# stecrotti/MPSKit.jl

Hardware: AMD Instinct MI355X
Metric: DMRG sweeps/sec + ddAC matvec achieved-TFLOP/s, Heisenberg L=100 D=1024 fp64 (higher is better)
Workload: dtype f64; 1 GPU; Heisenberg S=1/2 FiniteMPS L=100 D=1024 d=2 W=5 fp64, 1-site DMRG sweep (2L-2 site updates), fixed Krylov budget 8 matvecs/site; parallelism=single GPU

## Files before the change

mpskit.jl_amd/csrc/mpsk_api.hip:

```cpp
#include <hip/hip_runtime.h>
#include <cstdio>
#include <cstdlib>
#include <cstring>
#include <cmath>
#include <algorithm>
#include <map>
#include <string>
#include <vector>
#include "mpsk.h"
#include "mpsk_internal.h"

using namespace mpsk;

static thread_local std::string g_err;
static int fail(int code, const std::string& msg) { g_err = msg; return code; }
#define HIPCHK(expr)                                                                        \
  do {                                                                                      \
    hipError_t e_ = (expr);                                                                 \
    if (e_ != hipSuccess)                                                                   \
      return fail(MPSK_ERR_HIP, std::string(#expr) + ": " + hipGetErrorString(e_));         \
  } while (0)
#define REQUIRE(cond, msg)                                                  \
  do {                                                                      \
    if (!(cond)) return fail(MPSK_ERR_INVALID, std::string(__func__) + ": " + (msg)); \
// ... 12 lines not shown
  MixPlan rgt;
  double Oi(int w, int t, int s, int v) const {
    return Ofull_im.empty() ? 0.0 : Ofull_im[w + (size_t)Wl * (t + d * (s + (size_t)d * v))];
  }
  std::vector<char> row_used, col_used;
  MixPlan rc;
  std::vector<int> rc_w, rc_s, rc_t;
  int rc_nseg = 0;
  bool jordan = false;
  MixPlan jr, jl;
  std::vector<int> jr_p, jl_p;
  int jr_nseg = 0, jl_nseg = 0;
  MixPlan tl, tr;
  bool tl_dblock = false;
  mutable std::map<int64_t, int64_t*> jtabL;
  mutable std::map<std::pair<int64_t, int64_t>, int64_t*> jtabR;
  double O(int w, int t, int s, int v) const { return Ofull[w + (size_t)Wl * (t + d * (s + (size_t)d * v))]; }
  bool dense = false;
  double* d_Od = nullptr;
  mutable std::map<std::pair<int64_t, int64_t>, int64_t*> dtab;
  double* d_OdR = nullptr;
  mutable std::map<std::pair<int64_t, int64_t>, int64_t*> dtabR;
};

struct PoolBuf { void* p; size_t bytes; bool used; hipStream_t last = nullptr; hipEvent_t ev = nullptr; bool ev_set = false; };

struct mpsk_ctx {
  int device = 0;
  hipStream_t stream = nullptr;
  void* ws = nullptr;
  size_t ws_bytes = 0;
  double* d_scal = nullptr;
  double* d_partial = nullptr;
  double* h_scal = nullptr;
  double* d_coef = nullptr;
  double* h_coef = nullptr;
  hipEvent_t ev_coef = nullptr;
  bool coef_pending = false;
  int dtype = MPSK_F64;
  int last_svd_sweeps = 0;
  int split_skip = 0, split_backoff = 0;
  std::map<std::pair<int, int>, int> split_q_hint;
  int last_split_iters = 0, last_split_path = 0;
  double last_split_resid = 0.0;
  int svd_precondition = 3;
  int qr_mode = 0;
  int* d_flag = nullptr;
  long n_qr_chol = 0, n_qr_house = 0, n_qr_fallback = 0, n_qr_robust = 0, n_qr_retry = 0;
  double qr_shift_fast = getenv("MPSK_CQ_SHIFT_SCALE") ? atof(getenv("MPSK_CQ_SHIFT_SCALE")) : 1.0e-8;
  hipStream_t stream2 = nullptr;
  hipStream_t xstreams[3] = {nullptr, nullptr, nullptr};
  hipEvent_t ev_fork = nullptr, ev_join = nullptr;
  void* ws2 = nullptr;
  size_t ws2_bytes = 0;
  void* ws3 = nullptr;
  size_t ws3_bytes = 0;
  void* cxws[4] = {nullptr, nullptr, nullptr, nullptr};
  size_t cxws_bytes[4] = {0, 0, 0, 0};
  int* h_flags = nullptr;
  struct PendingQR {
    int active = 0;
    int m = 0, n = 0;
    const void *A1 = nullptr, *A2 = nullptr; void *Q1 = nullptr, *R1 = nullptr, *Q2 = nullptr, *R2 = nullptr;
    int lda1 = 0, ldq1 = 0, ldr1 = 0, lda2 = 0, ldq2 = 0, ldr2 = 0;
    double *At = nullptr, *Qt = nullptr, *Rt = nullptr, *ws = nullptr;
    void *L = nullptr, *Qo = nullptr; int ldl = 0, ldqo = 0;
// ... 15 lines not shown
  const double* GL;
  const double* GR;
  int mode;
  double* GRc = nullptr;
  double* GLc = nullptr;
  int launches = 1;
  int64_t* zseg = nullptr;
  std::vector<int64_t> zseg_host;
  hipEvent_t ev_up = nullptr;
  int pool_idx = -1;
};
constexpr int MAXK = 256;
constexpr int MAXCOEF = 1024;

extern "C" {

int mpsk_version(void) { return 100; }
const char* mpsk_last_error(void) { return g_err.c_str(); }

int mpsk_ctx_create(int device, mpsk_ctx** out) {
  REQUIRE(out != nullptr, "out is NULL");
  int ndev = 0;
  HIPCHK(hipGetDeviceCount(&ndev));
  REQUIRE(device >= 0 && device < ndev, "no such HIP device (is a GPU visible?)");
  HIPCHK(hipSetDevice(device));
  hipDeviceProp_t prop;
  HIPCHK(hipGetDeviceProperties(&prop, device));
  if (std::strncmp(prop.gcnArchName, "gfx950", 6) != 0)
    return fail(MPSK_ERR_UNSUPPORTED, std::string("libmpsk is built for gfx950 only, device is ") + prop.gcnArchName);
  mpsk_ctx* c = new mpsk_ctx();
  c->device = device;
  HIPCHK(hipMalloc(&c->d_scal, sizeof(double) * MAXK));
  HIPCHK(hipMalloc(&c->d_partial, sizeof(double) * MPSK_DOT_SCRATCH));
  HIPCHK(hipHostMalloc(&c->h_scal, sizeof(double) * MAXK, hipHostMallocDefault));
  HIPCHK(hipMalloc(&c->d_coef, sizeof(double) * MAXCOEF));
  HIPCHK(hipHostMalloc(&c->h_coef, sizeof(double) * MAXCOEF, hipHostMallocDefault));
  HIPCHK(hipEventCreateWithFlags(&c->ev_coef, hipEventDisableTiming | hipEventDisableSystemFence));
  HIPCHK(hipMalloc(&c->d_flag, 64));
  HIPCHK(hipHostMalloc(&c->h_flags, 64, hipHostMallocDefault));
  HIPCHK(hipStreamCreateWithFlags(&c->stream2, hipStreamNonBlocking));
  c->xstreams[0] = c->stream2;
  HIPCHK(hipStreamCreateWithFlags(&c->xstreams[1], hipStreamNonBlocking));
  HIPCHK(hipStreamCreateWithFlags(&c->xstreams[2], hipStreamNonBlocking));
  HIPCHK(hipEventCreateWithFlags(&c->ev_fork, hipEventDisableTiming | hipEventDisableSystemFence));
  HIPCHK(hipEventCreateWithFlags(&c->ev_join, hipEventDisableTiming | hipEventDisableSystemFence));
  gemm_retain_stream(c->stream);
  gemm_retain_stream(c->stream2);
  gemm_retain_stream(c->xstreams[1]);
  gemm_retain_stream(c->xstreams[2]);
  *out = c;
  return MPSK_OK;
}

int mpsk_ctx_destroy(mpsk_ctx* c) {
  if (!c) return MPSK_OK;
  (void)hipSetDevice(c->device);
  if (c->on_side) (void)mpsk_ctx_side_end(c);
  if (c->pend.active) (void)mpsk_qr_commit(c, nullptr);
  (void)hipStreamSynchronize(c->stream);
  if (c->stream2) (void)hipStreamSynchronize(c->stream2);
  gemm_release_stream(c->stream);
  gemm_release_stream(c->stream2);
  for (auto& kv : c->pair_plans) mix_plan_destroy(&kv.second);
  for (auto& b : c->pool) { if (b.p) (void)hipFree(b.p); if (b.ev) (void)hipEventDestroy(b.ev); }
  if (c->ws) (void)hipFree(c->ws);
  if (c->d_scal) (void)hipFree(c->d_scal);
  if (c->d_partial) (void)hipFree(c->d_partial);
  if (c->h_scal) (void)hipHostFree(c->h_scal);
  if (c->d_coef) (void)hipFree(c->d_coef);
  if (c->h_coef) (void)hipHostFree(c->h_coef);
  if (c->ev_coef) (void)hipEventDestroy(c->ev_coef);
  if (c->d_flag) (void)hipFree(c->d_flag);
  if (c->h_flags) (void)hipHostFree(c->h_flags);
  if (c->ws2) (void)hipFree(c->ws2);
  if (c->ws3) (void)hipFree(c->ws3);
  if (c->exws) (void)hipFree(c->exws);
  for (auto& kv : c->prod_tabs) (void)hipFree(kv.second);
  for (int i = 0; i < 4; ++i) if (c->cxws[i]) (void)hipFree(c->cxws[i]);
  for (int i = 1; i < 3; ++i)
    if (c->xstreams[i]) { (void)hipStreamSynchronize(c->xstreams[i]); gemm_release_stream(c->xstreams[i]); (void)hipStreamDestroy(c->xstreams[i]); }
  if (c->stream2) { (void)hipStreamSynchronize(c->stream2); (void)hipStreamDestroy(c->stream2); }
  if (c->ev_fork) (void)hipEventDestroy(c->ev_fork);
  if (c->ev_join) (void)hipEventDestroy(c->ev_join);
  delete c;
  return MPSK_OK;
}

int mpsk_ctx_set_stream(mpsk_ctx* c, void* s) {
  REQUIRE(c, "ctx is NULL");
  REQUIRE(!c->on_side, "not inside a side-stream section (mpsk_ctx_side_end first)");
  REQUIRE(!c->pend.active, "a deferred factorization is pending (mpsk_qr_commit first)");
  if (c->stream != (hipStream_t)s) {
    (void)hipSetDevice(c->device);
    (void)hipStreamSynchronize(c->stream);
    gemm_release_stream(c->stream);
    gemm_retain_stream((hipStream_t)s);
  }
  c->stream = (hipStream_t)s;
  return MPSK_OK;
}
// ... 969 lines not shown
  const bool cplx = h->H->dtype == MPSK_C128;
  const bool shift = a0[0] != 0.0 || (cplx && a0[1] != 0.0);
  const bool scale = a1[0] != 1.0 || (cplx && a1[1] != 0.0);
  REQUIRE(!shift || (h->Dlo == h->Dl && nblk == 1), "a shift needs a square operator (Dlo == Dl) on the plain vector layout");
  if (int rc = mpsk_hac_apply(h, x, nblk, y)) return rc;
  if (!shift && !scale) return MPSK_OK;
  mpsk_ctx* c = h->ctx;
  const int64_t n = (int64_t)h->Dlo * h->H->d * h->Dr;
  if (cplx) {
    HIPCHK(vec_axpby_c(a0, shift ? (const double*)x : nullptr, a1, (double*)y, n, c->stream));
  } else if (shift) {
    HIPCHK(vec_axpby(a0[0], (const double*)x, a1[0], (double*)y, n, c->stream));
  } else {
    HIPCHK(vec_scal(a1[0], (double*)y, n, c->stream));
  }
  return MPSK_OK;
}

int mpsk_hac_eigsolve_fixed(mpsk_hac* h, const void* x0, int m, void* const* V, void* scal, void* y, void* first_image) {
  REQUIRE(h && x0 && V && scal && y, "NULL argument");
  REQUIRE(m >= 1 && m <= 32, "needs 1 <= m <= 32");
  REQUIRE(h->H->dtype == MPSK_F64, "mpsk_hac_eigsolve_fixed: MPSK_F64 operators only");
  mpsk_ctx* c = h->ctx;
  HIPCHK(hipSetDevice(c->device));
  const int64_t n = (int64_t)h->Dlo * h->H->d * h->Dr;
  REQUIRE(h->Dlo == h->Dl, "mpsk_hac_eigsolve_fixed: the operator must be square (unsharded)");
  double* slot = (double*)scal;
  const int stride = 2 * m + 1;
  double* rbuf = slot + (size_t)m * stride;
  if (int rc = mpsk_vnormalize_dev(c, n, x0, V[0], nullptr)) return rc;
  for (int k = 0; k < m; ++k) {
    if (int rc = mpsk_hac_apply(h, V[k], 1, V[k + 1])) return rc;
    if (k == 0 && first_image) HIPCHK(hipMemcpyAsync(first_image, V[1], sizeof(double) * n, hipMemcpyDeviceToDevice, c->stream));
    HIPCHK(vec_cgs2((const double* const*)V, k + 1, (double*)V[k + 1], n, slot + (size_t)k * stride, c->d_partial, c->stream));
    HIPCHK(vec_scal_rsqrt_dev(slot + (size_t)k * stride + 2 * (k + 1), (double*)V[k + 1], n, c->stream));
  }
  HIPCHK(vec_ritz_small(slot, m, stride, rbuf, rbuf + 32, c->stream));
  HIPCHK(hipMemsetAsync(V[m + 1], 0, sizeof(double) * n, c->stream));
  HIPCHK(vec_multiaxpy((const double* const*)V, rbuf, m, 1.0, (double*)V[m + 1], n, c->stream));
  return mpsk_vnormalize_dev(c, n, V[m + 1], y, nullptr);
}

int mpsk_dC(mpsk_ctx* c, int W, int Dlo, int Dl, int Dr, const void* GL, const void* GR, const void* cm, void* y) {
  REQUIRE(c && GL && GR && cm && y, "NULL argument");
  REQUIRE(W > 0 && Dlo > 0 && Dl > 0 && Dr > 0, "dimensions must be positive");
  if (c->dtype == MPSK_C128)
    return dC_c128(c, W, Dlo, Dl, Dr, (const double*)GL, (const double*)GR, (const double*)cm, (double*)y);
  HIPCHK(hipSetDevice(c->device));
  const size_t slab = (size_t)Dlo * Dr;
  if (int rc = ensure_ws(c, sizeof(double) * slab * W)) return rc;
  double* T1 = (double*)c->ws;
  GemmArgs g1 = mk((const double*)GL, (const double*)cm, T1, Dlo, Dr, Dl, Dlo, Dl, Dlo);
  g1.batch = W; g1.bsA = (int64_t)Dlo * Dl; g1.bsB = 0; g1.bsC = (int64_t)slab;
  g1.tag = 1;
  HIPCHK(gemm_f64(g1, c->stream));
  std::vector<int64_t> sa, sb;
  for (int w = 0; w < W; ++w) { sa.push_back((int64_t)w * slab); sb.push_back((int64_t)w * Dr * Dr); }
  GemmArgs g3 = mk(T1, (const double*)GR, (double*)y, Dlo, Dr, Dr, Dlo, Dr, Dlo);
  g3.tag = 1;
  HIPCHK(gemm_segments(g3, sa, sb, c->stream));
  return MPSK_OK;
}

static int pair_plan(mpsk_ctx* c, const mpsk_mposlice* H1, const mpsk_mposlice* H2, const MixPlan** out) {
  auto key = std::make_pair(H1, H2);
  auto it = c->pair_plans.find(key);
  if (it != c->pair_plans.end()) { *out = &it->second; return MPSK_OK; }
  const int d1 = H1->d, d2 = H2->d, Wl = H1->Wl, Wm = H1->Wr, Wr = H2->Wr;
// ... 1417 lines not shown

int mpsk_vnrm2(mpsk_ctx* c, int64_t n, const void* x, double* host_out) {
  double v = 0.0;
  if (int rc = mpsk_vdot(c, n, x, x, &v)) return rc;
  *host_out = std::sqrt(v);
  return MPSK_OK;
}

int mpsk_vdiff_nrm2(mpsk_ctx* c, int64_t n, const void* x, const void* y, double* host_out) {
  REQUIRE(c && x && y && host_out, "NULL argument");
  REQUIRE(n > 0, "bad n");
  REQUIRE(((uintptr_t)x % 16 == 0) && ((uintptr_t)y % 16 == 0), "operands must be 16-byte aligned");
  HIPCHK(hipSetDevice(c->device));
  HIPCHK(vec_diff_nrm2((const double*)x, (const double*)y, c->dtype == MPSK_C128 ? 2 * n : n, c->d_scal, c->d_partial,
                       c->stream));
  return fetch_scalars(c, 2, host_out);
}

int mpsk_vgs_step(mpsk_ctx* c, int64_t n, int k, const void* const* xs, void* y, double* host_out) {
  REQUIRE(c && xs && y && host_out, "NULL argument");
  REQUIRE(k > 0 && k <= MAXK && n > 0, "bad k or n");
  HIPCHK(hipSetDevice(c->device));
  HIPCHK(vec_multidot((const double* const*)xs, k, (const double*)y, n, c->d_scal, c->d_partial, c->stream));
  HIPCHK(vec_multiaxpy((const double* const*)xs, c->d_scal, k, -1.0, (double*)y, n, c->stream));
  return fetch_scalars(c, k, host_out);
}

int mpsk_vorth_step(mpsk_ctx* c, int64_t n, int k, const void* const* xs, void* y, double* host_h, double* host_beta) {
  REQUIRE(c && xs && y && host_h && host_beta, "NULL argument");
  REQUIRE(k > 0 && 2 * k + 1 <= MAXK && n > 0, "bad k or n");
  HIPCHK(hipSetDevice(c->device));
  const double* const* X = (const double* const*)xs;
  double* yy = (double*)y;
  HIPCHK(vec_cgs2(X, k, yy, n, c->d_scal, c->d_partial, c->stream));
  HIPCHK(vec_scal_rsqrt_dev(c->d_scal + 2 * k, yy, n, c->stream));
  double tmp[MAXK];
  if (int rc = fetch_scalars(c, 2 * k + 1, tmp)) return rc;
  for (int j = 0; j < k; ++j) host_h[j] = tmp[j] + tmp[k + j];
  *host_beta = tmp[2 * k] > 0.0 ? std::sqrt(tmp[2 * k]) : 0.0;
  return MPSK_OK;
}

int mpsk_vorth_step_dev(mpsk_ctx* c, int64_t n, int k, const void* const* xs, void* y, void* dev_out) {
  REQUIRE(c && xs && y && dev_out, "NULL argument");
  REQUIRE(k > 0 && 2 * k + 1 <= MAXK && n > 0, "bad k or n");
  HIPCHK(hipSetDevice(c->device));
  const double* const* X = (const double* const*)xs;
  double* yy = (double*)y;
  double* out = (double*)dev_out;
  HIPCHK(vec_cgs2(X, k, yy, n, out, c->d_partial, c->stream));
  HIPCHK(vec_scal_rsqrt_dev(out + 2 * k, yy, n, c->stream));
  return MPSK_OK;
}

int mpsk_vlincomb(mpsk_ctx* c, int64_t n, int k, const void* const* xs, const double* host_coefs, void* y) {
  REQUIRE(c && xs && y && host_coefs, "NULL argument");
  REQUIRE(k > 0 && k <= MAXK && n > 0, "bad k or n");
  HIPCHK(hipSetDevice(c->device));
  if (c->coef_pending) { HIPCHK(hipEventSynchronize(c->ev_coef)); c->coef_pending = false; }
  std::memcpy(c->h_coef, host_coefs, sizeof(double) * k);
  HIPCHK(hipMemcpyAsync(c->d_coef, c->h_coef, sizeof(double) * k, hipMemcpyHostToDevice, c->stream));
  HIPCHK(hipEventRecord(c->ev_coef, c->stream));
  c->coef_pending = true;
  HIPCHK(hipMemsetAsync(y, 0, sizeof(double) * n, c->stream));
  HIPCHK(vec_multiaxpy((const double* const*)xs, c->d_coef, k, 1.0, (double*)y, n, c->stream));
  return MPSK_OK;
}

int mpsk_vmultilincomb(mpsk_ctx* c, int64_t n, int k, const void* const* xs, int m, void* const* ys, const double* host_coefs) {
  REQUIRE(c && xs && ys && host_coefs, "NULL argument");
  REQUIRE(k > 0 && k <= 32 && m > 0 && m <= 32 && n > 0, "needs 0 < k, m <= 32 and n > 0");
  for (int j = 0; j < m; ++j)
    for (int i = 0; i < k; ++i) REQUIRE(ys[j] != xs[i], "outputs must not alias inputs");
  HIPCHK(hipSetDevice(c->device));
  if (c->coef_pending) { HIPCHK(hipEventSynchronize(c->ev_coef)); c->coef_pending = false; }
  std::memcpy(c->h_coef, host_coefs, sizeof(double) * (size_t)k * m);
  HIPCHK(hipMemcpyAsync(c->d_coef, c->h_coef, sizeof(double) * (size_t)k * m, hipMemcpyHostToDevice, c->stream));
  HIPCHK(hipEventRecord(c->ev_coef, c->stream));
  c->coef_pending = true;
  HIPCHK(vec_multilincomb((const double* const*)xs, k, (double* const*)ys, m, c->d_coef, n, c->stream));
  return MPSK_OK;
}

int mpsk_vritz_dev(mpsk_ctx* c, int m, int stride, const void* dev_slot, void* dev_coef, void* dev_info) {
  REQUIRE(c && dev_slot && dev_coef, "NULL argument");
  REQUIRE(m > 0 && m <= 32 && stride >= 2 * m + 1, "needs 0 < m <= 32 and stride >= 2 m + 1");
  HIPCHK(hipSetDevice(c->device));
  HIPCHK(vec_ritz_small((const double*)dev_slot, m, stride, (double*)dev_coef, (double*)dev_info, c->stream));
  return MPSK_OK;
}

int mpsk_vlincomb_dev(mpsk_ctx* c, int64_t n, int k, const void* const* xs, const void* dev_coefs, void* y) {
  REQUIRE(c && xs && y && dev_coefs, "NULL argument");
  REQUIRE(k > 0 && k <= MAXK && n > 0, "bad k or n");
  HIPCHK(hipSetDevice(c->device));
  HIPCHK(hipMemsetAsync(y, 0, sizeof(double) * n, c->stream));
  HIPCHK(vec_multiaxpy((const double* const*)xs, (const double*)dev_coefs, k, 1.0, (double*)y, n, c->stream));
  return MPSK_OK;
}

int mpsk_vnormalize_dev(mpsk_ctx* c, int64_t n, const void* x, void* y, void* dev_n2) {
  REQUIRE(c && x && y, "NULL argument");
  REQUIRE(n > 0, "bad n");
  HIPCHK(hipSetDevice(c->device));
  double* n2 = dev_n2 ? (double*)dev_n2 : c->d_scal + (MAXK - 1);
  const double* xs[1] = {(const double*)x};
  HIPCHK(vec_multidot(xs, 1, (const double*)x, n, n2, c->d_partial, c->stream));
  if (y != x) HIPCHK(vec_scal_rsqrt_dev_oop(n2, (const double*)x, (double*)y, n, c->stream));
  else HIPCHK(vec_scal_rsqrt_dev(n2, (double*)y, n, c->stream));
  return MPSK_OK;
}

int mpsk_vnrm2_dev(mpsk_ctx* c, int64_t n, const void* x, void* dev_out) {
  REQUIRE(c && x && dev_out, "NULL argument");
  REQUIRE(n > 0, "bad n");
  HIPCHK(hipSetDevice(c->device));
  const double* xs[1] = {(const double*)x};
  HIPCHK(vec_multidot(xs, 1, (const double*)x, n, (double*)dev_out, c->d_partial, c->stream));
  return MPSK_OK;
}

int mpsk_vaxpby(mpsk_ctx* c, int64_t n, double alpha, const void* x, double beta, void* y) {
  REQUIRE(c && x && y, "NULL argument");
  HIPCHK(hipSetDevice(c->device));
  HIPCHK(vec_axpby(alpha, (const double*)x, beta, (double*)y, n, c->stream));
  return MPSK_OK;
}
static bool aligned16(const void* p) { return (uintptr_t)p % 16 == 0; }

int mpsk_vdotc(mpsk_ctx* c, int64_t n, const void* x, const void* y, double* host_out) {
  REQUIRE(c && x && y && host_out, "NULL argument");
  REQUIRE(n > 0, "bad n");
  REQUIRE(aligned16(x) && aligned16(y), "operands must be 16-byte aligned");
  HIPCHK(hipSetDevice(c->device));
  const double* xs[1] = {(const double*)x};
  HIPCHK(vec_multidotc(xs, 1, (const double*)y, n, c->d_scal, c->d_partial, c->stream));
  return fetch_scalars(c, 2, host_out);
}

int mpsk_vaxpby_c(mpsk_ctx* c, int64_t n, const double* alpha, const void* x, const double* beta, void* y) {
  REQUIRE(c && x && y && alpha && beta, "NULL argument");
  REQUIRE(n > 0, "bad n");
// ... 359 lines not shown
```

mpskit.jl_amd/csrc/mpsk_internal.h:

```cpp
#pragma once
#include <hip/hip_runtime.h>
#include <stdint.h>
#include <stddef.h>
#include <atomic>
#include <vector>
#include <string>

namespace mpsk {

inline hipError_t ensure_dyn_smem(std::atomic<uint64_t>& done, const void* kernel, size_t bytes) {
  int dev = 0;
  hipError_t e = hipGetDevice(&dev);
  if (e != hipSuccess) return e;
  const uint64_t bit = 1ull << (dev & 63);
  if (done.load(std::memory_order_acquire) & bit) return hipSuccess;
  e = hipFuncSetAttribute(kernel, hipFuncAttributeMaxDynamicSharedMemorySize, (int)bytes);
  if (e != hipSuccess) return e;
  done.fetch_or(bit, std::memory_order_release);
  return hipSuccess;
}

constexpr int MAXSEG = 32;

struct GemmArgs {
// ... 59 lines not shown

struct MixTerm { int32_t out, in; double coef; double coef_im = 0.0; };

struct MixPlan {
  int n_out = 0, n_in = 0;
  int32_t* d_rowptr = nullptr;
  int32_t* d_src = nullptr;
  double* d_coef = nullptr;
  double* d_coef_im = nullptr;
  int nnz = 0;
  int max_terms = 0;
};

hipError_t mix_plan_create(const std::vector<MixTerm>& terms, int n_out, int n_in, MixPlan* plan);
void mix_plan_destroy(MixPlan* plan);

struct SlabIndex { int n0, n1; int64_t s0, s1, s2; int64_t ld; };
hipError_t mix_apply(const MixPlan& plan, const double* in, SlabIndex iin, double* out, SlabIndex iout,
                     int R, int C, hipStream_t s);
hipError_t deinterleave(const double* z, int64_t n, double* re, double* im, hipStream_t s);
hipError_t copy_strided(const double* src, int64_t srs, int64_t scs, double* dst, int64_t drs, int64_t dcs, int64_t R,
                        int64_t C, hipStream_t s);
hipError_t identity_slab(double* G, int n, hipStream_t s);

constexpr int MPSK_DOT_SCRATCH = 32 * 1024;
hipError_t vec_multidot(const double* const* xs, int k, const double* y, int64_t n, double* d_out,
                        double* d_partial, hipStream_t s);
hipError_t vec_diff_nrm2(const double* x, const double* y, int64_t n, double* d_out, double* d_partial, hipStream_t s);
hipError_t vec_axpby(double a, const double* x, double b, double* y, int64_t n, hipStream_t s);
hipError_t vec_times_i(const double* x, double* y, int64_t n, hipStream_t s);
hipError_t vec_scal(double a, double* x, int64_t n, hipStream_t s);
hipError_t vec_scal_rsqrt_dev(const double* d_n2, double* x, int64_t n, hipStream_t s);
hipError_t vec_scal_rsqrt_dev_oop(const double* d_n2, const double* x, double* y, int64_t n, hipStream_t s);
hipError_t vec_cgs2(const double* const* xs, int k, double* y, int64_t n, double* d_out, double* d_partial, hipStream_t s);
hipError_t vec_ritz_small(const double* d_slot, int m, int stride, double* d_coef, double* d_info, hipStream_t s);
hipError_t vec_multilincomb(const double* const* xs, int k, double* const* ys, int m, const double* d_coefs, int64_t n,
                            hipStream_t s);
hipError_t vec_multiaxpy(const double* const* xs, const double* d_coefs, int k, double sign, double* y,
                         int64_t n, hipStream_t s);
hipError_t vec_multidotc(const double* const* xs, int k, const double* y, int64_t n, double* d_out, double* d_partial,
                         hipStream_t s);
hipError_t vec_multiaxpy_c(const double* const* xs, const double* d_coefs, int k, double sign, double* y, int64_t n,
                           hipStream_t s);
hipError_t vec_cgs2_c(const double* const* xs, int k, double* y, int64_t n, double* d_out, double* d_partial, hipStream_t s);
hipError_t vec_axpby_c(const double a[2], const double* x, const double b[2], double* y, int64_t n, hipStream_t s);
hipError_t identity_dev_c(const double* G, int n, double* d_out, int nblocks, hipStream_t s);

size_t regularize_workspace_doubles(int W, int D1, int D2);
hipError_t regularize(int W, int D1, int D2, double* v, const double* lvec, const double* rvec, double* partial, hipStream_t s);
hipError_t transpose(const double* in, int ldi, int rows, int cols, double* out, int ldo, hipStream_t s);
size_t qrpos_workspace_doubles(int m, int n);
hipError_t qrpos(int m, int n, const double* A, int lda, double* Q, int ldq, double* R, int ldr, double* ws,
                 hipStream_t s, std::string* err);

size_t cholqr_workspace_doubles(int m, int n);
hipError_t cholqr3(int m, int n, const double* A, int lda, double* Q, int ldq, double* R, int ldr, double* ws,
                   int* d_flag, int* flag_out, hipStream_t s, double shift_scale = 1.0);
hipError_t cholqr_robust(int m, int n, const double* A, int lda, double* Q, int ldq, double* R, int ldr, double* ws,
                         int* d_flag, int* flag_out, hipStream_t s);
hipError_t cholqr1_orth(int m, int n, const double* X, int ldx, double* Q, int ldq, double* ws, int* d_flag, hipStream_t s,
                        double shift_scale);
hipError_t cholqr3_enqueue(int m, int n, const double* A, int lda, double* Q, int ldq, double* R, int ldr, double* ws,
                           int* d_flag, int* flag_out, hipStream_t s, double shift_scale = 1.0);
hipError_t cholqr3_finalize(int m, int n, double* Q, int ldq, double* R, int ldr, double* ws, int* d_flag,
                            int* flag_out, hipStream_t s);
size_t tsvd_workspace_bytes(int m, int n);
hipError_t tsvd(int m, int n, const double* theta, int ldt, double* U, int ldu, double* S, double* Vh, int ldv,
// ... 10 lines not shown
```

mpskit.jl_amd/csrc/mpsk_ops.hip:

```cpp
#include <hip/hip_runtime.h>
#include "mpsk_internal.h"

namespace mpsk {

typedef double d2 __attribute__((ext_vector_type(2)));

__device__ inline int64_t slab_off(const SlabIndex& ix, int j) {
  int j0 = j % ix.n0;
  int t = j / ix.n0;
  int j1 = t % ix.n1;
  int j2 = t / ix.n1;
  return j0 * ix.s0 + j1 * ix.s1 + j2 * ix.s2;
}

template <bool VEC2>
__global__ __launch_bounds__(256) void mix_kernel(const int32_t* __restrict__ rowptr,
                                                  const int32_t* __restrict__ src,
                                                  const double* __restrict__ coef,
                                                  const double* __restrict__ coef_im,
                                                  const double* __restrict__ in, SlabIndex iin,
                                                  double* __restrict__ out, SlabIndex iout, int R, int C) {
  const int o = blockIdx.y;
  const int t0 = rowptr[o], t1 = rowptr[o + 1];
  double* op = out + slab_off(iout, o);
  if (VEC2) {
    const int R2 = R >> 1;
    const int64_t total = (int64_t)R2 * C;
    for (int64_t e = blockIdx.x * (int64_t)blockDim.x + threadIdx.x; e < total;
         e += (int64_t)gridDim.x * blockDim.x) {
      int r = (int)(e % R2) * 2, c = (int)(e / R2);
      d2 acc = {0.0, 0.0};
      if (coef_im) {
        for (int t = t0; t < t1; ++t) {
// ... 172 lines not shown
    for (int j = 0; j < NVEC; ++j) {
      d2 xv = *reinterpret_cast<const d2*>(xs.p[j] + 2 * e);
      acc[j] += xv.x * yv.x + xv.y * yv.y;
    }
  }
  if ((n & 1) && blockIdx.x == 0 && threadIdx.x == 0) {
#pragma unroll
    for (int j = 0; j < NVEC; ++j) acc[j] += xs.p[j][n - 1] * y[n - 1];
  }
  block_sum<NVEC>(acc, sh);
  if (threadIdx.x == 0) {
#pragma unroll
    for (int j = 0; j < NVEC; ++j) partial[(int64_t)j * DOT_BLOCKS + blockIdx.x] = acc[j];
  }
}

__global__ __launch_bounds__(256) void dot_final_kernel(const double* __restrict__ partial, int nblocks,
                                                        double* __restrict__ out) {
  __shared__ double sh[4];
  double acc[1] = {0.0};
  const double* p = partial + (int64_t)blockIdx.x * DOT_BLOCKS;
  for (int i = threadIdx.x; i < nblocks; i += blockDim.x) acc[0] += p[i];
  block_sum<1>(acc, sh);
  if (threadIdx.x == 0) out[blockIdx.x] = acc[0];
}

static int dot_grid(int64_t n) {
  int64_t b = (n / 2 + 255) / 256;
  if (b < 1) b = 1;
  if (b > DOT_BLOCKS) b = DOT_BLOCKS;
  return (int)b;
}

hipError_t vec_multidot(const double* const* xs, int k, const double* y, int64_t n, double* d_out,
                        double* d_partial, hipStream_t s) {
  const int nb = dot_grid(n);
  for (int j0 = 0; j0 < k; j0 += MD) {
    int nv = k - j0 < MD ? k - j0 : MD;
    PtrPack pk;
    for (int j = 0; j < MD; ++j) pk.p[j] = xs[j0 + (j < nv ? j : 0)];
    switch (nv) {
      case 1: hipLaunchKernelGGL(multidot_kernel<1>, dim3(nb), dim3(256), 0, s, pk, y, n, d_partial); break;
      case 2: hipLaunchKernelGGL(multidot_kernel<2>, dim3(nb), dim3(256), 0, s, pk, y, n, d_partial); break;
      case 3: hipLaunchKernelGGL(multidot_kernel<3>, dim3(nb), dim3(256), 0, s, pk, y, n, d_partial); break;
      case 4: hipLaunchKernelGGL(multidot_kernel<4>, dim3(nb), dim3(256), 0, s, pk, y, n, d_partial); break;
      case 5: hipLaunchKernelGGL(multidot_kernel<5>, dim3(nb), dim3(256), 0, s, pk, y, n, d_partial); break;
      case 6: hipLaunchKernelGGL(multidot_kernel<6>, dim3(nb), dim3(256), 0, s, pk, y, n, d_partial); break;
      case 7: hipLaunchKernelGGL(multidot_kernel<7>, dim3(nb), dim3(256), 0, s, pk, y, n, d_partial); break;
      default: hipLaunchKernelGGL(multidot_kernel<8>, dim3(nb), dim3(256), 0, s, pk, y, n, d_partial); break;
    }
    hipLaunchKernelGGL(dot_final_kernel, dim3(nv), dim3(256), 0, s, d_partial, nb, d_out + j0);
  }
  return hipGetLastError();
}

__global__ __launch_bounds__(256) void diff_nrm2_kernel(const double* __restrict__ x, const double* __restrict__ y, int64_t n,
                                                        double* __restrict__ partial) {
  __shared__ double sh[4 * 2];
  double acc[2] = {0.0, 0.0};
  const int64_t n2 = n >> 1;
  for (int64_t e = blockIdx.x * (int64_t)blockDim.x + threadIdx.x; e < n2; e += (int64_t)gridDim.x * blockDim.x) {
    const d2 xv = *reinterpret_cast<const d2*>(x + 2 * e);
    const d2 yv = *reinterpret_cast<const d2*>(y + 2 * e);
    const double d0 = xv.x - yv.x, d1 = xv.y - yv.y;
    acc[0] += d0 * d0 + d1 * d1;
    acc[1] += xv.x * xv.x + xv.y * xv.y;
// ... 47 lines not shown
  if ((n & 1) && blockIdx.x == 0 && threadIdx.x == 0) {
    double v = y[n - 1];
#pragma unroll
    for (int j = 0; j < NVEC; ++j) v += c[j] * xs.p[j][n - 1];
    y[n - 1] = v;
    if (NORM) acc[0] += v * v;
    else {
#pragma unroll
      for (int j = 0; j < NVEC; ++j) acc[NORM ? 0 : j] += xs.p[j][n - 1] * v;
    }
  }
  block_sum<NA>(acc, sh);
  if (threadIdx.x == 0) {
#pragma unroll
    for (int j = 0; j < NA; ++j) partial[(int64_t)j * DOT_BLOCKS + blockIdx.x] = acc[j];
  }
}

template <bool NORM>
static void launch_axpy_dot(int nv, int nb, const PtrPack& pk, const double* cf, double sign, double* y, int64_t n,
                            double* d_partial, hipStream_t s) {
  switch (nv) {
    case 1: hipLaunchKernelGGL((multiaxpy_dot_kernel<1, NORM>), dim3(nb), dim3(256), 0, s, pk, cf, sign, y, n, d_partial); break;
    case 2: hipLaunchKernelGGL((multiaxpy_dot_kernel<2, NORM>), dim3(nb), dim3(256), 0, s, pk, cf, sign, y, n, d_partial); break;
    case 3: hipLaunchKernelGGL((multiaxpy_dot_kernel<3, NORM>), dim3(nb), dim3(256), 0, s, pk, cf, sign, y, n, d_partial); break;
    case 4: hipLaunchKernelGGL((multiaxpy_dot_kernel<4, NORM>), dim3(nb), dim3(256), 0, s, pk, cf, sign, y, n, d_partial); break;
    case 5: hipLaunchKernelGGL((multiaxpy_dot_kernel<5, NORM>), dim3(nb), dim3(256), 0, s, pk, cf, sign, y, n, d_partial); break;
    case 6: hipLaunchKernelGGL((multiaxpy_dot_kernel<6, NORM>), dim3(nb), dim3(256), 0, s, pk, cf, sign, y, n, d_partial); break;
    case 7: hipLaunchKernelGGL((multiaxpy_dot_kernel<7, NORM>), dim3(nb), dim3(256), 0, s, pk, cf, sign, y, n, d_partial); break;
    default: hipLaunchKernelGGL((multiaxpy_dot_kernel<8, NORM>), dim3(nb), dim3(256), 0, s, pk, cf, sign, y, n, d_partial); break;
  }
}

constexpr int ML = 32;
struct PtrPackL { const double* p[ML]; };

template <int NVEC>
__global__ __launch_bounds__(256) void multiaxpy_dot_long_kernel(PtrPackL xs, const double* __restrict__ coefs, double sign,
                                                                 double* __restrict__ y, int64_t n, int k,
                                                                 double* __restrict__ partial) {
  __shared__ double sh[4 * NVEC];
  double c[NVEC], acc[NVEC];
#pragma unroll
  for (int j = 0; j < NVEC; ++j) { c[j] = j < k ? sign * coefs[j] : 0.0; acc[j] = 0.0; }
  for (int64_t e = blockIdx.x * (int64_t)blockDim.x + threadIdx.x; e < n; e += (int64_t)gridDim.x * blockDim.x) {
    double yv = y[e];
    double xv[NVEC];
#pragma unroll
    for (int j = 0; j < NVEC; ++j) {
      xv[j] = xs.p[j][e];
      yv += c[j] * xv[j];
    }
    y[e] = yv;
#pragma unroll
    for (int j = 0; j < NVEC; ++j) acc[j] += xv[j] * yv;
  }
  block_sum<NVEC>(acc, sh);
  if (threadIdx.x == 0) {
#pragma unroll
    for (int j = 0; j < NVEC; ++j)
      if (j < k) partial[(int64_t)j * DOT_BLOCKS + blockIdx.x] = acc[j];
  }
}

__global__ __launch_bounds__(256) void multiaxpy_norm_long_kernel(PtrPackL xs, const double* __restrict__ coefs, double sign,
                                                                  double* __restrict__ y, int64_t n, int k,
                                                                  double* __restrict__ partial) {
  __shared__ double sh[4];
  __shared__ double cs[ML];
  if (threadIdx.x < ML) cs[threadIdx.x] = threadIdx.x < k ? sign * coefs[threadIdx.x] : 0.0;
  __syncthreads();
  double acc[1] = {0.0};
  for (int64_t e = blockIdx.x * (int64_t)blockDim.x + threadIdx.x; e < n; e += (int64_t)gridDim.x * blockDim.x) {
    double yv = y[e];
    for (int j = 0; j < k; ++j) yv += cs[j] * xs.p[j][e];
    y[e] = yv;
    acc[0] += yv * yv;
  }
  block_sum<1>(acc, sh);
  if (threadIdx.x == 0) partial[blockIdx.x] = acc[0];
}

static int dot_grid_long(int64_t n) {
  int64_t b = (n + 255) / 256;
  if (b < 1) b = 1;
  if (b > DOT_BLOCKS) b = DOT_BLOCKS;
  return (int)b;
}

hipError_t vec_cgs2(const double* const* xs, int k, double* y, int64_t n, double* d_out, double* d_partial, hipStream_t s) {
  if (n <= 0 || k <= 0) return hipErrorInvalidValue;
  hipError_t e = vec_multidot(xs, k, y, n, d_out, d_partial, s);
  if (e != hipSuccess) return e;
  if (k > MD && k <= ML) {
    const int nbl = dot_grid_long(n);
    PtrPackL pk;
    for (int j = 0; j < ML; ++j) pk.p[j] = xs[j < k ? j : 0];
    if (k <= 16) hipLaunchKernelGGL(multiaxpy_dot_long_kernel<16>, dim3(nbl), dim3(256), 0, s, pk, d_out, -1.0, y, n, k, d_partial);
    else if (k <= 24) hipLaunchKernelGGL(multiaxpy_dot_long_kernel<24>, dim3(nbl), dim3(256), 0, s, pk, d_out, -1.0, y, n, k, d_partial);
    else hipLaunchKernelGGL(multiaxpy_dot_long_kernel<32>, dim3(nbl), dim3(256), 0, s, pk, d_out, -1.0, y, n, k, d_partial);
    hipLaunchKernelGGL(dot_final_kernel, dim3(k), dim3(256), 0, s, d_partial, nbl, d_out + k);
    hipLaunchKernelGGL(multiaxpy_norm_long_kernel, dim3(nbl), dim3(256), 0, s, pk, d_out + k, -1.0, y, n, k, d_partial);
    hipLaunchKernelGGL(dot_final_kernel, dim3(1), dim3(256), 0, s, d_partial, nbl, d_out + 2 * k);
    return hipGetLastError();
  }
  if (k > MD) {
    if ((e = vec_multiaxpy(xs, d_out, k, -1.0, y, n, s)) != hipSuccess) return e;
    if ((e = vec_multidot(xs, k, y, n, d_out + k, d_partial, s)) != hipSuccess) return e;
    if ((e = vec_multiaxpy(xs, d_out + k, k, -1.0, y, n, s)) != hipSuccess) return e;
    const double* ys[1] = {y};
    return vec_multidot(ys, 1, y, n, d_out + 2 * k, d_partial, s);
  }
  const int nb = dot_grid(n);
  PtrPack pk;
  for (int j = 0; j < MD; ++j) pk.p[j] = xs[j < k ? j : 0];
  launch_axpy_dot<false>(k, nb, pk, d_out, -1.0, y, n, d_partial, s);
  hipLaunchKernelGGL(dot_final_kernel, dim3(k), dim3(256), 0, s, d_partial, nb, d_out + k);
  launch_axpy_dot<true>(k, nb, pk, d_out + k, -1.0, y, n, d_partial, s);
  hipLaunchKernelGGL(dot_final_kernel, dim3(1), dim3(256), 0, s, d_partial, nb, d_out + 2 * k);
  return hipGetLastError();
}

__global__ __launch_bounds__(256) void axpby_kernel(double a, const double* __restrict__ x, double b,
                                                    double* __restrict__ y, int64_t n) {
// ... 17 lines not shown
  for (int64_t e = blockIdx.x * (int64_t)blockDim.x + threadIdx.x; e < npairs; e += (int64_t)gridDim.x * blockDim.x) {
    const d2 v = reinterpret_cast<const d2*>(x)[e];
    reinterpret_cast<d2*>(y)[e] = d2{-v.y, v.x};
  }
}
hipError_t vec_times_i(const double* x, double* y, int64_t n, hipStream_t s) {
  const int64_t npairs = n / 2;
  int64_t nb = (npairs + 255) / 256;
  if (nb > 4096) nb = 4096;
  if (nb < 1) nb = 1;
  hipLaunchKernelGGL(times_i_kernel, dim3((int)nb), dim3(256), 0, s, x, y, npairs);
  return hipGetLastError();
}

__global__ __launch_bounds__(256) void scal_kernel(double a, double* x, int64_t n) {
  for (int64_t e = blockIdx.x * (int64_t)blockDim.x + threadIdx.x; e < n; e += (int64_t)gridDim.x * blockDim.x)
    x[e] *= a;
}

__global__ __launch_bounds__(256) void scal_rsqrt_dev_kernel(const double* __restrict__ d_n2, double* x, int64_t n) {
  const double n2 = *d_n2;
  const double a = (n2 > 0.0) ? 1.0 / sqrt(n2) : 0.0;
  for (int64_t e = blockIdx.x * (int64_t)blockDim.x + threadIdx.x; e < n; e += (int64_t)gridDim.x * blockDim.x)
    x[e] *= a;
}

__global__ __launch_bounds__(256) void scal_rsqrt_dev_oop_kernel(const double* __restrict__ d_n2, const double* __restrict__ x,
                                                                 double* __restrict__ y, int64_t n) {
  const double n2 = *d_n2;
  const double a = (n2 > 0.0) ? 1.0 / sqrt(n2) : 0.0;
  for (int64_t e = blockIdx.x * (int64_t)blockDim.x + threadIdx.x; e < n; e += (int64_t)gridDim.x * blockDim.x)
    y[e] = a * x[e];
}
hipError_t vec_scal_rsqrt_dev_oop(const double* d_n2, const double* x, double* y, int64_t n, hipStream_t s) {
  if (n <= 0) return hipSuccess;
  int64_t nb = (n + 255) / 256;
  if (nb > 4096) nb = 4096;
  hipLaunchKernelGGL(scal_rsqrt_dev_oop_kernel, dim3((int)nb), dim3(256), 0, s, d_n2, x, y, n);
  return hipGetLastError();
}

hipError_t vec_scal_rsqrt_dev(const double* d_n2, double* x, int64_t n, hipStream_t s) {
  if (n <= 0) return hipSuccess;
  int64_t nb = (n + 255) / 256;
  if (nb > 4096) nb = 4096;
  hipLaunchKernelGGL(scal_rsqrt_dev_kernel, dim3((int)nb), dim3(256), 0, s, d_n2, x, n);
  return hipGetLastError();
}

constexpr int RITZ_MAX = 32;
__device__ __forceinline__ double ritz_rcp(double x) {
  double r = __builtin_amdgcn_rcp(x);
  r = r * (2.0 - x * r);
  return r * (2.0 - x * r);
}
__device__ __forceinline__ double ritz_rsq(double x) {
  double r = __builtin_amdgcn_rsq(x);
  r = r * (1.5 - 0.5 * x * r * r);
  return r * (1.5 - 0.5 * x * r * r);
}
__global__ __launch_bounds__(64) void ritz_small_kernel(const double* __restrict__ slot, int m, int stride,
                                                        double* __restrict__ coef, double* __restrict__ info) {
  __shared__ double A[RITZ_MAX][RITZ_MAX + 1], V[RITZ_MAX][RITZ_MAX + 1], beta[RITZ_MAX];
  __shared__ int meff_s, rp[RITZ_MAX / 2], rq[RITZ_MAX / 2];
  __shared__ double rc[RITZ_MAX / 2], rs[RITZ_MAX / 2];
  const int t = threadIdx.x;
// ... 352 lines not shown
```

Baseline: 1.152 sweeps/s.

## Fuse dot-product final reductions into consumer kernels for Krylov orthogonalization

Separate dot_final reduction launches are removed from the CGS2 orthogonalization and normalize paths. Each consumer kernel (axpy+dot, axpy+norm, scale) now reduces the previous kernel's per-block partials itself, and triple-buffered partial scratch sets avoid read/write hazards between kernels. This cuts kernel launches and serialization per Krylov step for small k. The cost is that every block redundantly re-reduces up to DOT_BLOCKS partials. An env var can turn the new path off.

```diff
diff --git a/mpskit.jl_amd/csrc/mpsk_api.hip b/mpskit.jl_amd/csrc/mpsk_api.hip
--- a/mpskit.jl_amd/csrc/mpsk_api.hip
+++ b/mpskit.jl_amd/csrc/mpsk_api.hip
@@ -68,6 +68,7 @@
   size_t ws_bytes = 0;
   double* d_scal = nullptr;
   double* d_partial = nullptr;
+  double* d_pset[3] = {nullptr, nullptr, nullptr};
   double* h_scal = nullptr;
   double* d_coef = nullptr;
   double* h_coef = nullptr;
@@ -149,6 +150,9 @@
   c->device = device;
   HIPCHK(hipMalloc(&c->d_scal, sizeof(double) * MAXK));
   HIPCHK(hipMalloc(&c->d_partial, sizeof(double) * MPSK_DOT_SCRATCH));
+  HIPCHK(hipMalloc(&c->d_pset[1], sizeof(double) * 2 * MPSK_DOT_SET));
+  c->d_pset[0] = c->d_partial;
+  c->d_pset[2] = c->d_pset[1] + MPSK_DOT_SET;
   HIPCHK(hipHostMalloc(&c->h_scal, sizeof(double) * MAXK, hipHostMallocDefault));
   HIPCHK(hipMalloc(&c->d_coef, sizeof(double) * MAXCOEF));
   HIPCHK(hipHostMalloc(&c->h_coef, sizeof(double) * MAXCOEF, hipHostMallocDefault));
@@ -183,6 +187,7 @@
   if (c->ws) (void)hipFree(c->ws);
   if (c->d_scal) (void)hipFree(c->d_scal);
   if (c->d_partial) (void)hipFree(c->d_partial);
+  if (c->d_pset[1]) (void)hipFree(c->d_pset[1]);
   if (c->h_scal) (void)hipHostFree(c->h_scal);
   if (c->d_coef) (void)hipFree(c->d_coef);
   if (c->h_coef) (void)hipHostFree(c->h_coef);
@@ -1218,8 +1223,7 @@
   for (int k = 0; k < m; ++k) {
     if (int rc = mpsk_hac_apply(h, V[k], 1, V[k + 1])) return rc;
     if (k == 0 && first_image) HIPCHK(hipMemcpyAsync(first_image, V[1], sizeof(double) * n, hipMemcpyDeviceToDevice, c->stream));
-    HIPCHK(vec_cgs2((const double* const*)V, k + 1, (double*)V[k + 1], n, slot + (size_t)k * stride, c->d_partial, c->stream));
-    HIPCHK(vec_scal_rsqrt_dev(slot + (size_t)k * stride + 2 * (k + 1), (double*)V[k + 1], n, c->stream));
+    HIPCHK(vec_orth_step((const double* const*)V, k + 1, (double*)V[k + 1], n, slot + (size_t)k * stride, c->d_pset, c->stream));
   }
   HIPCHK(vec_ritz_small(slot, m, stride, rbuf, rbuf + 32, c->stream));
   HIPCHK(hipMemsetAsync(V[m + 1], 0, sizeof(double) * n, c->stream));
@@ -2703,8 +2707,7 @@
   HIPCHK(hipSetDevice(c->device));
   const double* const* X = (const double* const*)xs;
   double* yy = (double*)y;
-  HIPCHK(vec_cgs2(X, k, yy, n, c->d_scal, c->d_partial, c->stream));
-  HIPCHK(vec_scal_rsqrt_dev(c->d_scal + 2 * k, yy, n, c->stream));
+  HIPCHK(vec_orth_step(X, k, yy, n, c->d_scal, c->d_pset, c->stream));
   double tmp[MAXK];
   if (int rc = fetch_scalars(c, 2 * k + 1, tmp)) return rc;
   for (int j = 0; j < k; ++j) host_h[j] = tmp[j] + tmp[k + j];
@@ -2719,8 +2722,7 @@
   const double* const* X = (const double* const*)xs;
   double* yy = (double*)y;
   double* out = (double*)dev_out;
-  HIPCHK(vec_cgs2(X, k, yy, n, out, c->d_partial, c->stream));
-  HIPCHK(vec_scal_rsqrt_dev(out + 2 * k, yy, n, c->stream));
+  HIPCHK(vec_orth_step(X, k, yy, n, out, c->d_pset, c->stream));
   return MPSK_OK;
 }
 
@@ -2775,10 +2777,7 @@
   REQUIRE(n > 0, "bad n");
   HIPCHK(hipSetDevice(c->device));
   double* n2 = dev_n2 ? (double*)dev_n2 : c->d_scal + (MAXK - 1);
-  const double* xs[1] = {(const double*)x};
-  HIPCHK(vec_multidot(xs, 1, (const double*)x, n, n2, c->d_partial, c->stream));
-  if (y != x) HIPCHK(vec_scal_rsqrt_dev_oop(n2, (const double*)x, (double*)y, n, c->stream));
-  else HIPCHK(vec_scal_rsqrt_dev(n2, (double*)y, n, c->stream));
+  HIPCHK(vec_normalize((const double*)x, (double*)y, n, n2, c->d_partial, c->stream));
   return MPSK_OK;
 }
 
diff --git a/mpskit.jl_amd/csrc/mpsk_internal.h b/mpskit.jl_amd/csrc/mpsk_internal.h
--- a/mpskit.jl_amd/csrc/mpsk_internal.h
+++ b/mpskit.jl_amd/csrc/mpsk_internal.h
@@ -115,7 +115,13 @@
 hipError_t vec_scal(double a, double* x, int64_t n, hipStream_t s);
 hipError_t vec_scal_rsqrt_dev(const double* d_n2, double* x, int64_t n, hipStream_t s);
 hipError_t vec_scal_rsqrt_dev_oop(const double* d_n2, const double* x, double* y, int64_t n, hipStream_t s);
-hipError_t vec_cgs2(const double* const* xs, int k, double* y, int64_t n, double* d_out, double* d_partial, hipStream_t s);
+constexpr int MPSK_DOT_SET = 8 * 1024;
+hipError_t vec_cgs2(const double* const* xs, int k, double* y, int64_t n, double* d_out, double* const d_pset[3],
+                    const double** n2_part, hipStream_t s);
+hipError_t vec_scal_rsqrt_part(const double* d_part, double* d_n2, const double* x, double* y, int64_t n, hipStream_t s);
+hipError_t vec_orth_step(const double* const* xs, int k, double* y, int64_t n, double* d_out, double* const d_pset[3],
+                         hipStream_t s);
+hipError_t vec_normalize(const double* x, double* y, int64_t n, double* d_n2, double* d_partial, hipStream_t s);
 hipError_t vec_ritz_small(const double* d_slot, int m, int stride, double* d_coef, double* d_info, hipStream_t s);
 hipError_t vec_multilincomb(const double* const* xs, int k, double* const* ys, int m, const double* d_coefs, int64_t n,
                             hipStream_t s);
diff --git a/mpskit.jl_amd/csrc/mpsk_ops.hip b/mpskit.jl_amd/csrc/mpsk_ops.hip
--- a/mpskit.jl_amd/csrc/mpsk_ops.hip
+++ b/mpskit.jl_amd/csrc/mpsk_ops.hip
@@ -1,4 +1,5 @@
 #include <hip/hip_runtime.h>
+#include <cstdlib>
 #include "mpsk_internal.h"
 
 namespace mpsk {
@@ -237,6 +238,55 @@
   return (int)b;
 }
 
+constexpr int PART_TRIPS = DOT_BLOCKS / 256;
+template <int NV>
+__device__ inline void partial_load(const double* __restrict__ partial, int nblocks, double (&pv)[NV][PART_TRIPS]) {
+#pragma unroll
+  for (int r = 0; r < PART_TRIPS; ++r) {
+    const int i = threadIdx.x + 256 * r;
+#pragma unroll
+    for (int v = 0; v < NV; ++v) pv[v][r] = i < nblocks ? partial[(int64_t)v * DOT_BLOCKS + i] : 0.0;
+  }
+}
+template <int NV>
+__device__ inline void partial_sums(const double (&pv)[NV][PART_TRIPS], int nblocks, double* sh ,
+                                    double* sums ) {
+  double acc[NV];
+#pragma unroll
+  for (int v = 0; v < NV; ++v) acc[v] = 0.0;
+#pragma unroll
+  for (int r = 0; r < PART_TRIPS; ++r) {
+    if (threadIdx.x + 256 * r < nblocks) {
+#pragma unroll
+      for (int v = 0; v < NV; ++v) acc[v] += pv[v][r];
+    }
+  }
+  block_sum<NV>(acc, sh);
+  if (threadIdx.x == 0) {
+#pragma unroll
+    for (int v = 0; v < NV; ++v) sums[v] = acc[v];
+  }
+  __syncthreads();
+}
+
+static bool consumer_final() {
+  static const bool enabled = !(getenv("MPSK_VEC_FINAL") && atoi(getenv("MPSK_VEC_FINAL")) == 1);
+  return enabled;
+}
+
+static void launch_multidot(int nv, int nb, const PtrPack& pk, const double* y, int64_t n, double* d_partial, hipStream_t s) {
+  switch (nv) {
+    case 1: hipLaunchKernelGGL(multidot_kernel<1>, dim3(nb), dim3(256), 0, s, pk, y, n, d_partial); break;
+    case 2: hipLaunchKernelGGL(multidot_kernel<2>, dim3(nb), dim3(256), 0, s, pk, y, n, d_partial); break;
+    case 3: hipLaunchKernelGGL(multidot_kernel<3>, dim3(nb), dim3(256), 0, s, pk, y, n, d_partial); break;
+    case 4: hipLaunchKernelGGL(multidot_kernel<4>, dim3(nb), dim3(256), 0, s, pk, y, n, d_partial); break;
+    case 5: hipLaunchKernelGGL(multidot_kernel<5>, dim3(nb), dim3(256), 0, s, pk, y, n, d_partial); break;
+    case 6: hipLaunchKernelGGL(multidot_kernel<6>, dim3(nb), dim3(256), 0, s, pk, y, n, d_partial); break;
+    case 7: hipLaunchKernelGGL(multidot_kernel<7>, dim3(nb), dim3(256), 0, s, pk, y, n, d_partial); break;
+    default: hipLaunchKernelGGL(multidot_kernel<8>, dim3(nb), dim3(256), 0, s, pk, y, n, d_partial); break;
+  }
+}
+
 hipError_t vec_multidot(const double* const* xs, int k, const double* y, int64_t n, double* d_out,
                         double* d_partial, hipStream_t s) {
   const int nb = dot_grid(n);
@@ -350,6 +400,78 @@
   }
 }
 
+template <int NVEC, bool NORM>
+__global__ __launch_bounds__(256) void multiaxpy_dot_cf_kernel(PtrPack xs, const double* __restrict__ cpart, int cnb,
+                                                               double* __restrict__ coefs_out, double sign,
+                                                               double* __restrict__ y, int64_t n, double* __restrict__ partial) {
+  constexpr int NA = NORM ? 1 : NVEC;
+  __shared__ double sh[4 * NVEC];
+  __shared__ double coefs[NVEC];
+  double pv[NVEC][PART_TRIPS];
+  partial_load<NVEC>(cpart, cnb, pv);
+  const int64_t n2 = n >> 1;
+  int64_t e = blockIdx.x * (int64_t)blockDim.x + threadIdx.x;
+  d2 yv = {0.0, 0.0}, xv[NVEC];
+  if (e < n2) {
+    yv = *reinterpret_cast<const d2*>(y + 2 * e);
+#pragma unroll
+    for (int j = 0; j < NVEC; ++j) xv[j] = *reinterpret_cast<const d2*>(xs.p[j] + 2 * e);
+  }
+  partial_sums<NVEC>(pv, cnb, sh, coefs);
+  if (blockIdx.x == 0 && threadIdx.x < NVEC) coefs_out[threadIdx.x] = coefs[threadIdx.x];
+  double c[NVEC], acc[NA];
+#pragma unroll
+  for (int j = 0; j < NVEC; ++j) c[j] = sign * coefs[j];
+#pragma unroll
+  for (int j = 0; j < NA; ++j) acc[j] = 0.0;
+  for (bool first = true; e < n2; e += (int64_t)gridDim.x * blockDim.x, first = false) {
+    if (!first) yv = *reinterpret_cast<const d2*>(y + 2 * e);
+#pragma unroll
+    for (int j = 0; j < NVEC; ++j) {
+      if (!first) xv[j] = *reinterpret_cast<const d2*>(xs.p[j] + 2 * e);
+      yv.x += c[j] * xv[j].x;
+      yv.y += c[j] * xv[j].y;
+    }
+    *reinterpret_cast<d2*>(y + 2 * e) = yv;
+    if (NORM) acc[0] += yv.x * yv.x + yv.y * yv.y;
+    else {
+#pragma unroll
+      for (int j = 0; j < NVEC; ++j) acc[NORM ? 0 : j] += xv[j].x * yv.x + xv[j].y * yv.y;
+    }
+  }
+  if ((n & 1) && blockIdx.x == 0 && threadIdx.x == 0) {
+    double v = y[n - 1];
+#pragma unroll
+    for (int j = 0; j < NVEC; ++j) v += c[j] * xs.p[j][n - 1];
+    y[n - 1] = v;
+    if (NORM) acc[0] += v * v;
+    else {
+#pragma unroll
+      for (int j = 0; j < NVEC; ++j) acc[NORM ? 0 : j] += xs.p[j][n - 1] * v;
+    }
+  }
+  block_sum<NA>(acc, sh);
+  if (threadIdx.x == 0) {
+#pragma unroll
+    for (int j = 0; j < NA; ++j) partial[(int64_t)j * DOT_BLOCKS + blockIdx.x] = acc[j];
+  }
+}
+
+template <bool NORM>
+static void launch_axpy_dot_cf(int nv, int nb, const PtrPack& pk, const double* cpart, double* cf_out, double sign, double* y,
+                               int64_t n, double* d_partial, hipStream_t s) {
+  switch (nv) {
+    case 1: hipLaunchKernelGGL((multiaxpy_dot_cf_kernel<1, NORM>), dim3(nb), dim3(256), 0, s, pk, cpart, nb, cf_out, sign, y, n, d_partial); break;
+    case 2: hipLaunchKernelGGL((multiaxpy_dot_cf_kernel<2, NORM>), dim3(nb), dim3(256), 0, s, pk, cpart, nb, cf_out, sign, y, n, d_partial); break;
+    case 3: hipLaunchKernelGGL((multiaxpy_dot_cf_kernel<3, NORM>), dim3(nb), dim3(256), 0, s, pk, cpart, nb, cf_out, sign, y, n, d_partial); break;
+    case 4: hipLaunchKernelGGL((multiaxpy_dot_cf_kernel<4, NORM>), dim3(nb), dim3(256), 0, s, pk, cpart, nb, cf_out, sign, y, n, d_partial); break;
+    case 5: hipLaunchKernelGGL((multiaxpy_dot_cf_kernel<5, NORM>), dim3(nb), dim3(256), 0, s, pk, cpart, nb, cf_out, sign, y, n, d_partial); break;
+    case 6: hipLaunchKernelGGL((multiaxpy_dot_cf_kernel<6, NORM>), dim3(nb), dim3(256), 0, s, pk, cpart, nb, cf_out, sign, y, n, d_partial); break;
+    case 7: hipLaunchKernelGGL((multiaxpy_dot_cf_kernel<7, NORM>), dim3(nb), dim3(256), 0, s, pk, cpart, nb, cf_out, sign, y, n, d_partial); break;
+    default: hipLaunchKernelGGL((multiaxpy_dot_cf_kernel<8, NORM>), dim3(nb), dim3(256), 0, s, pk, cpart, nb, cf_out, sign, y, n, d_partial); break;
+  }
+}
+
 constexpr int ML = 32;
 struct PtrPackL { const double* p[ML]; };
 
@@ -406,8 +528,21 @@
   return (int)b;
 }
 
-hipError_t vec_cgs2(const double* const* xs, int k, double* y, int64_t n, double* d_out, double* d_partial, hipStream_t s) {
+hipError_t vec_cgs2(const double* const* xs, int k, double* y, int64_t n, double* d_out, double* const d_pset[3],
+                    const double** n2_part, hipStream_t s) {
   if (n <= 0 || k <= 0) return hipErrorInvalidValue;
+  *n2_part = nullptr;
+  double* const d_partial = d_pset[0];
+  if (k <= MD && consumer_final()) {
+    const int nb = dot_grid(n);
+    PtrPack pk;
+    for (int j = 0; j < MD; ++j) pk.p[j] = xs[j < k ? j : 0];
+    launch_multidot(k, nb, pk, y, n, d_pset[0], s);
+    launch_axpy_dot_cf<false>(k, nb, pk, d_pset[0], d_out, -1.0, y, n, d_pset[1], s);
+    launch_axpy_dot_cf<true>(k, nb, pk, d_pset[1], d_out + k, -1.0, y, n, d_pset[2], s);
+    *n2_part = d_pset[2];
+    return hipGetLastError();
+  }
   hipError_t e = vec_multidot(xs, k, y, n, d_out, d_partial, s);
   if (e != hipSuccess) return e;
   if (k > MD && k <= ML) {
@@ -491,6 +626,72 @@
   for (int64_t e = blockIdx.x * (int64_t)blockDim.x + threadIdx.x; e < n; e += (int64_t)gridDim.x * blockDim.x)
     y[e] = a * x[e];
 }
+__global__ __launch_bounds__(256) void scal_rsqrt_part_kernel(const double* __restrict__ part, int pnb, double* __restrict__ d_n2,
+                                                              double* x, int64_t n) {
+  __shared__ double sh[4], sum[1];
+  double pv[1][PART_TRIPS];
+  partial_load<1>(part, pnb, pv);
+  int64_t e = blockIdx.x * (int64_t)blockDim.x + threadIdx.x;
+  double xv = e < n ? x[e] : 0.0;
+  partial_sums<1>(pv, pnb, sh, sum);
+  const double n2 = sum[0];
+  if (blockIdx.x == 0 && threadIdx.x == 0) *d_n2 = n2;
+  const double a = (n2 > 0.0) ? 1.0 / sqrt(n2) : 0.0;
+  for (bool first = true; e < n; e += (int64_t)gridDim.x * blockDim.x, first = false) {
+    if (!first) xv = x[e];
+    x[e] = xv * a;
+  }
+}
+__global__ __launch_bounds__(256) void scal_rsqrt_part_oop_kernel(const double* __restrict__ part, int pnb,
+                                                                  double* __restrict__ d_n2, const double* __restrict__ x,
+                                                                  double* __restrict__ y, int64_t n) {
+  __shared__ double sh[4], sum[1];
+  double pv[1][PART_TRIPS];
+  partial_load<1>(part, pnb, pv);
+  int64_t e = blockIdx.x * (int64_t)blockDim.x + threadIdx.x;
+  double xv = e < n ? x[e] : 0.0;
+  partial_sums<1>(pv, pnb, sh, sum);
+  const double n2 = sum[0];
+  if (blockIdx.x == 0 && threadIdx.x == 0) *d_n2 = n2;
+  const double a = (n2 > 0.0) ? 1.0 / sqrt(n2) : 0.0;
+  for (bool first = true; e < n; e += (int64_t)gridDim.x * blockDim.x, first = false) {
+    if (!first) xv = x[e];
+    y[e] = a * xv;
+  }
+}
+hipError_t vec_scal_rsqrt_part(const double* d_part, double* d_n2, const double* x, double* y, int64_t n, hipStream_t s) {
+  if (n <= 0) return hipSuccess;
+  int64_t nb = (n + 255) / 256;
+  if (nb > 4096) nb = 4096;
+  const int pnb = dot_grid(n);
+  if (y != x) hipLaunchKernelGGL(scal_rsqrt_part_oop_kernel, dim3((int)nb), dim3(256), 0, s, d_part, pnb, d_n2, x, y, n);
+  else hipLaunchKernelGGL(scal_rsqrt_part_kernel, dim3((int)nb), dim3(256), 0, s, d_part, pnb, d_n2, y, n);
+  return hipGetLastError();
+}
+
+hipError_t vec_orth_step(const double* const* xs, int k, double* y, int64_t n, double* d_out, double* const d_pset[3],
+                         hipStream_t s) {
+  const double* n2_part = nullptr;
+  hipError_t e = vec_cgs2(xs, k, y, n, d_out, d_pset, &n2_part, s);
+  if (e != hipSuccess) return e;
+  if (n2_part) return vec_scal_rsqrt_part(n2_part, d_out + 2 * k, y, y, n, s);
+  return vec_scal_rsqrt_dev(d_out + 2 * k, y, n, s);
+}
+
+hipError_t vec_normalize(const double* x, double* y, int64_t n, double* d_n2, double* d_partial, hipStream_t s) {
+  if (n <= 0) return hipErrorInvalidValue;
+  if (consumer_final()) {
+    PtrPack pk;
+    for (int j = 0; j < MD; ++j) pk.p[j] = x;
+    launch_multidot(1, dot_grid(n), pk, x, n, d_partial, s);
+    return vec_scal_rsqrt_part(d_partial, d_n2, x, y, n, s);
+  }
+  const double* xs[1] = {x};
+  hipError_t e = vec_multidot(xs, 1, x, n, d_n2, d_partial, s);
+  if (e != hipSuccess) return e;
+  return y != x ? vec_scal_rsqrt_dev_oop(d_n2, x, y, n, s) : vec_scal_rsqrt_dev(d_n2, y, n, s);
+}
+
 hipError_t vec_scal_rsqrt_dev_oop(const double* d_n2, const double* x, double* y, int64_t n, hipStream_t s) {
   if (n <= 0) return hipSuccess;
   int64_t nb = (n + 255) / 256;
```

Result: no change. 1.163 sweeps/s, median of 6 (+0.9%).
